# agimus-project/agimus_controller

Hardware: AMD Instinct MI355X
Metric: MPC steps/sec (horizon=100, Panda 7-DoF) (higher is better)
Workload: dtype f64; 1 GPU; Panda 7-DoF sine_wave_configuration_space, ocp_goal_reaching.yaml costs, horizon=100, dt=0.01, batch=1024 independent MPC instances per GPU (seed 1234+b), closed loop on own prediction; horizon=100, batch_per_gpu=1024, global_batch=1024, max_iter=10

## Files before the change

### agimus_controller_amd/csrc/agimus_hip.hip

```cpp

#include <hip/hip_runtime.h>

#include <algorithm>
#include <chrono>
#include <climits>
#include <cmath>
#include <cstddef>
#include <cstdio>
#include <cstdlib>
#include <cstring>
#include <string>
#include <vector>

#include "agx_kernels.hpp"

extern "C" int agx_cost_pairs_launch(int dest, void *stream, long long nodes, const DevModel *m, const DevOcp *o, const DevCostWide *w,
                                     const double *dts, const double *xs, const RefView *rv, double *out, double *auxs, const DevState *st,
                                     int phase, int sel, int which, const void *obs);
extern "C" int agx_cost_pairs_fill_launch(void *stream, const DevCostWide *w, const double *gw_item, double *traj, long long units, int stride);
extern "C" int agx_cost_pairs_fill_ring_launch(void *stream, const DevCostWide *w, const double *gw_item, double *traj, int B, int m_new, int end,
                                               int cap, int mirror, int stride);
extern "C" int agx_diag_iter_log_launch(void *stream, const DevState *st, int B, int it, int phase, agx_iter_record *rec, int *n, int capacity);
extern "C" int agx_diag_item_costs_launch(void *stream, int nv, int chain, const DevModel *m, const DevRows *rows2, int B, int T, const double *xs,
                                          const double *us, const RefView *rv, int R, double *cost, double *Lx, double *Lu, const void *obs);
// ... 359 lines not shown
      HIPCHK(hipGetLastError());
      return 0;
    }
    if constexpr (NV <= 7) {
      if (pair && o->riccati_mx && !forward)
        hipLaunchKernelGGL((agx::k_riccati_mx_pair_sweeps<NV>), dim3(16 * ((o->B + 7) / 8)), dim3(64), 0, o->stream, o->d_ocp, o->d_dt, o->d_qt,
                           o->d_aux, o->d_Kws, o->d_kws, o->d_dx, o->d_w, o->d_Kout, o->d_state, iter);
      else if (pair && o->riccati_mx)
        hipLaunchKernelGGL((agx::k_riccati_mx_pair<NV>), dim3(16 * ((o->B + 7) / 8)), dim3(64), 0, o->stream, o->d_ocp, o->d_dt, o->d_qt, o->d_aux,
                           o->d_Kws, o->d_kws, o->d_dx, o->d_w, o->d_Kout, o->d_state, iter);
      else if (pair)
        hipLaunchKernelGGL((agx::k_riccati_pair<NV>), dim3(2 * o->B), dim3(64), 0, o->stream, o->d_ocp, o->d_dt, o->d_qt, o->d_aux,
                           o->d_Kws, o->d_kws, o->d_dx, o->d_w, o->d_du, o->d_Kout, o->d_state, iter);
      else if (o->riccati_mx)
        hipLaunchKernelGGL((agx::k_riccati_mx<NV, false>), dim3(o->B), dim3(64), 0, o->stream, o->d_ocp, o->d_dt, qt, o->d_aux,
                           o->d_Kws, o->d_kws, o->d_dx, o->d_w, o->d_Kout, o->d_state, forward, 0);
      else
        hipLaunchKernelGGL((agx::k_riccati<NV, false>), dim3(o->B), dim3(64), 0, o->stream, o->d_ocp, o->d_dt, qt, o->d_aux,
                           o->d_Kws, o->d_kws, o->d_dx, o->d_w, o->d_du, o->d_Kout, o->d_state, forward, 0);
    } else {
      (void)pair; (void)iter;
      launch_riccati_blk<NV>(o, qt, forward, 0);
    }
    HIPCHK(hipGetLastError());
    return 0;
  });
}

agx::HostWords host_words(agx_ocp *o, bool line_search_counters, unsigned long long seq) {
  agx::HostWords hw{nullptr, nullptr, nullptr, nullptr, nullptr, nullptr, 0};
  if (!o->poll || !o->fold_publish || seq == 0) return hw;
  hw.done = o->h_ndone_dev + 0;
  if (line_search_counters) { hw.handed = o->h_ndone_dev + 6; hw.stale = o->h_ndone_dev + 7; }
  hw.carry = o->h_ndone_dev + 8;
  hw.packed = o->h_ndone_dev + 9;
  hw.seq = o->h_ndone_dev + 1;
  hw.stamp = seq;
  return hw;
}

double *first_block(const agx_ocp *o) {
  return (o->first_in_solve && o->poll && o->first_stride == o->nu + o->nu * o->nx + o->nx + 8) ? o->d_first : nullptr;
}

int launch_step(agx_ocp *o, int iter, int max_iter, int mode, bool with_node_kkt = true, bool with_step = true, unsigned long long seq = 0,
                bool pack = false) {
  if (o->T + 1 > 512) return fail("step kernel supports horizons up to 511 nodes");
  return dispatch(o->nv, o->chain, [&](auto NVc, auto CHc) -> int {
    constexpr int NV = decltype(NVc)::value;
    constexpr bool CH = decltype(CHc)::value;
    (void)CH;
    const long long nodes = (long long)o->B * (o->T + 1);
    double *xs_t = o->d_xs + (size_t)o->B * (o->T + 1) * o->nx, *us_t = o->d_us + (size_t)o->B * o->T * o->nu;
    if (with_node_kkt) {
      if constexpr (NV <= 7) {
        if (o->general)
          hipLaunchKernelGGL((agx::k_node_kkt_gen<NV>), dim3((int)((nodes + 63) / 64)), dim3(64), 0, o->stream, o->d_ocp, o->d_qt, o->d_aux,
                             o->d_auxg, o->d_dx, o->d_w, o->d_du, o->d_nodestat, o->d_state);
        else if (o->node_kkt_wide)
          hipLaunchKernelGGL((agx::k_node_kkt_ahead<NV>), dim3((int)((nodes + 7) / 8)), dim3(64), 0, o->stream, o->d_ocp, o->d_qt, o->d_aux,
                             o->d_dx, o->d_w, o->d_du, o->d_nodestat, o->d_state);
        else
          hipLaunchKernelGGL((agx::k_node_kkt<NV>), dim3((int)((nodes * 8 + 255) / 256)), dim3(256), 0, o->stream, o->d_ocp, o->d_qt, o->d_aux,
                             o->d_dx, o->d_w, o->d_du, o->d_nodestat, o->d_state);
      } else if (kGeneralRowsWg && o->general)
        HIPCHK((hipError_t)agx_general_kkt_launch((void *)o->stream, NV, nodes, o->d_ocp, o->d_qt, o->d_aux, o->d_auxg, o->d_dx, o->d_w, o->d_du,
                                                  o->d_nodestat, o->d_state));
      else
        hipLaunchKernelGGL((agx::k_node_kkt_big<NV>), dim3((int)((nodes + 1) / 2)), dim3(64), 0, o->stream, o->d_ocp, o->d_qt, o->d_aux,
                           o->d_dx, o->d_w, o->d_du, o->d_nodestat, o->d_state);
    }
    if (with_step)
      hipLaunchKernelGGL((agx::k_sqp_head<NV>), dim3(o->B), dim3(128), 0, o->stream, o->d_ocp, o->d_xs, o->d_us, o->d_dx, o->d_du, xs_t, us_t,
                         o->d_nodestat, o->d_state, iter, max_iter, mode, o->d_ndone, host_words(o, false, seq), o->d_Kout,
                         pack ? first_block(o) : nullptr, o->first_stride);
    HIPCHK(hipGetLastError());
    return 0;
  });
}

bool step_tail_path(const agx_ocp *o) {
  return o->step_tail && o->nv <= 7 && !o->has_con && !o->general && o->riccati_mx && o->node_kkt_wide && o->mx2_S < 2;
}
int launch_step_tail(agx_ocp *o, int iter, int max_iter, unsigned long long seq, bool pack) {
  if (o->T + 1 > 512) return fail("step kernel supports horizons up to 511 nodes");
  return dispatch(o->nv, o->chain, [&](auto NVc, auto CHc) -> int {
    constexpr int NV = decltype(NVc)::value;
    (void)CHc;
    if constexpr (NV <= 7) {
      double *xs_t = o->d_xs + (size_t)o->B * (o->T + 1) * o->nx, *us_t = o->d_us + (size_t)o->B * o->T * o->nu;
      hipLaunchKernelGGL((agx::k_step_tail<NV>), dim3(o->B), dim3(agx::kTailThreads), 0, o->stream, o->d_ocp, o->d_dt, o->d_qt, o->d_aux,
                         o->d_Kws, o->d_kws, o->d_xs, o->d_us, o->d_dx, o->d_w, o->d_du, xs_t, us_t, o->d_nodestat, o->d_state, iter,
                         max_iter, o->d_ndone, host_words(o, false, seq), o->d_Kout, pack ? first_block(o) : nullptr, o->first_stride);
      HIPCHK(hipGetLastError());
      o->step_tail_launches += 1;
      return 0;
    } else {
      (void)iter; (void)max_iter; (void)seq; (void)pack;
      return fail("the step tail serves the 7-joint capacity");
    }
  });
}

int launch_gains(agx_ocp *o, int gmode = 0) {
  if (o->nv <= 7 && o->T + 1 > 512) return fail("the sweeps stage the step lengths of up to 511 nodes in LDS: horizon too long");
  if (o->nv > 7 && !o->d_qt2) HIPCHK(o->own.device(&o->d_qt2, (size_t)o->B * (o->T + 1) * o->qt_size));
  return dispatch(o->nv, o->chain, [&](auto NVc, auto CHc) -> int {
    constexpr int NV = decltype(NVc)::value;
    if constexpr (NV <= 7) {
      if (o->riccati_mx)
        hipLaunchKernelGGL((agx::k_riccati_mx<NV, true>), dim3(o->B), dim3(64), 0, o->stream, o->d_ocp, o->d_dt, o->d_qt, o->d_aux, o->d_Kws,
                           o->d_kws, o->d_dx, o->d_w, o->d_Kout, o->d_state, 0, gmode);
      else
      hipLaunchKernelGGL((agx::k_riccati<NV, true>), dim3(o->B), dim3(64), 0, o->stream, o->d_ocp, o->d_dt, o->d_qt, o->d_aux, o->d_Kws,
                         o->d_kws, o->d_dx, o->d_w, o->d_du, o->d_Kout, o->d_state, 0, gmode);
    } else {
      const long long nodes = (long long)o->B * (o->T + 1);
      const int gsel = gmode == 0 ? 1 : gmode;
      hipLaunchKernelGGL((agx::k_sigma_tile_big<NV>), dim3((int)nodes), dim3(256), 0, o->stream, o->d_ocp, o->d_qt, o->d_qt2, o->d_aux);
      launch_riccati_blk<NV>(o, o->d_qt2, 0, gsel);
      if constexpr (NV > 16) {
        if (o->gains_mfma) {
          hipLaunchKernelGGL((agx::k_gains_to_u_mfma<NV>), dim3(o->B * o->T), dim3(64), 0, o->stream, o->d_ocp, o->d_aux, o->d_Kws, o->d_Kout,
                             o->d_state);
          HIPCHK(hipGetLastError());
          return 0;
        }
      }
      const long long units = (long long)o->B * o->T * 64;
      hipLaunchKernelGGL((agx::k_gains_to_u_big<NV>), dim3((int)((units + 255) / 256)), dim3(256), 0, o->stream, o->d_ocp, o->d_aux,
                         o->d_Kws, o->d_Kout, o->d_state);
    }
    HIPCHK(hipGetLastError());
    return 0;
  });
}

int reset_state(agx_ocp *o) {
  hipLaunchKernelGGL(agx::k_reset_state, dim3((o->B + 255) / 256), dim3(256), 0, o->stream, o->d_state, o->B, o->d_ndone);
  HIPCHK(hipGetLastError());
  return 0;
}

int launch_rollout(agx_ocp *o, int n_substeps, double dt_sub, const double *d_dist) {
  return dispatch(o->nv, o->chain, [&](auto NVc, auto CHc) -> int {
    constexpr int NV = decltype(NVc)::value;
    constexpr bool CH = decltype(CHc)::value;
    if (o->plant_set || o->minert_set)
      hipLaunchKernelGGL((agx::k_plant_rollout<NV, CH>), dim3((o->B + 63) / 64), dim3(64), 0, o->stream, o->d_model,
                         (const agx::PlantInertials<NV> *)(o->plant_set ? o->d_plant : o->d_minert), o->d_us, o->d_Kout, o->d_x0, d_dist, o->B, o->T,
                         n_substeps, dt_sub);
    else
      hipLaunchKernelGGL((agx::k_feedback_rollout<NV, CH>), dim3((o->B + 63) / 64), dim3(64), 0, o->stream, o->d_model, o->d_us, o->d_Kout, o->d_x0,
                         d_dist, o->B, o->T, n_substeps, dt_sub);
    HIPCHK(hipGetLastError());
    return 0;
  });
}

int prof_mark(agx_ocp *o, int kind, bool start) {
  if (!o->prof) return 0;
  if (o->prof_used == o->prof_ev.size()) {
    o->prof_ev.push_back(nullptr);
    HIPCHK(o->own.event(&o->prof_ev.back()));
  }
  HIPCHK(hipEventRecord(o->prof_ev[o->prof_used++], o->stream));
  if (start) o->prof_kind.push_back(kind);
  return 0;
}
int prof_collect(agx_ocp *o) {
  if (!o->prof || o->prof_used == 0) return 0;
  HIPCHK(hipStreamSynchronize(o->stream));
  for (size_t k = 0; k < o->prof_kind.size(); ++k) {
    float ms = 0.f;
    HIPCHK(hipEventElapsedTime(&ms, o->prof_ev[2 * k], o->prof_ev[2 * k + 1]));
    o->prof_ms[o->prof_kind[k]] += ms;
// ... 1895 lines not shown
```

### agimus_controller_amd/csrc/agx_host_handle.hpp

```cpp
#pragma once

#include <deque>

namespace {

thread_local std::string g_err;
int fail(const std::string &msg) {
  g_err = msg;
  return -1;
}
#define HIPCHK(expr)                                                                                      \
  do {                                                                                                    \
    hipError_t e_ = (expr);                                                                               \
    if (e_ != hipSuccess) return fail(std::string(#expr) + ": " + hipGetErrorString(e_));                \
  } while (0)

class DeviceOwner {
 public:
  DeviceOwner() = default;
  DeviceOwner(const DeviceOwner &) = delete;
  ~DeviceOwner() { for (const Held &h : held_) free_value(*h.field, h.kind); }
  template <class T> hipError_t device(T **field, size_t count, bool zero = false) { return device_bytes((void **)field, sizeof(T) * count, zero); }
  hipError_t device_bytes(void **field, size_t bytes, bool zero = false) {
    void *p = nullptr;
// ... 11 lines not shown
    const hipError_t e = hipEventCreateWithFlags(&ev, flags);
    return adopt((void **)field, (void *)ev, kEvent, e);
  }
  template <class T> void release(T *field) {
    for (Held &h : held_)
      if (h.field == (void **)field) {
        free_value(*h.field, h.kind);
        *h.field = nullptr;
        h = held_.back();
        held_.pop_back();
        return;
      }
  }

 private:
  enum Kind { kDevice, kPinned, kEvent };
  struct Held { void **field; Kind kind; };
  static void free_value(void *p, Kind kind) {
    if (p) (void)(kind == kDevice ? hipFree(p) : (kind == kPinned ? hipHostFree(p) : hipEventDestroy((hipEvent_t)p)));
  }
  hipError_t adopt(void **field, void *p, Kind kind, hipError_t e) {
    if (e != hipSuccess) return e;
    release(field);
    *field = p;
    held_.push_back({field, kind});
    return hipSuccess;
  }
  std::vector<Held> held_;
};

}

struct agx_model {
  DevModel h;
  int nvu = 0;
};

struct agx_ocp {
  DevModel hm;
  DevOcp ho;
  int nv = 0, nx = 0, nu = 0, T = 0, B = 0, tile = 0, stride = 0, device = 0;
  int nvu = 0, stride_u = 0;
  bool padded = false;
  std::vector<int> refmap[2];
  std::vector<double> reffill[2];
  std::vector<double> stage;
  std::vector<double> h_first_u;
  bool chain = false;
  std::vector<double> dt;
  hipStream_t stream = nullptr;
  bool own_stream = false;
  DevModel *d_model = nullptr;
  DevOcp *d_ocp = nullptr;
  double *d_dt = nullptr, *d_xs = nullptr, *d_us = nullptr, *d_x0 = nullptr, *d_tiles = nullptr;
  double *d_Kws = nullptr, *d_kws = nullptr, *d_Kout = nullptr, *d_dx = nullptr, *d_du = nullptr;
  double *d_Kws_lqr = nullptr, *d_kws_lqr = nullptr;
  bool admm_prefactor = true;
  double *d_qt = nullptr, *d_aux = nullptr, *d_w = nullptr, *d_nodestat = nullptr;
  bool has_con = false;
  std::vector<int> shift_nodes;
  int *d_shift_nodes = nullptr;
  bool general = false;
  double *d_auxg = nullptr;
  double *d_qt2 = nullptr, *d_cg = nullptr, *d_cjac = nullptr, *d_y = nullptr, *d_z = nullptr, *d_cx = nullptr, *d_admmstat = nullptr,
         *d_fac = nullptr,
         *d_segP = nullptr;
  bool admm_segments = true;
  int qt_size = 0, aux_size = 0;
  bool k1_lanes = true;
  bool lanes_ok = true;
  bool lanes_coll = false;
  bool cost_wide = false;
  DevCostWide hw{};
  DevCostWide *d_cw = nullptr;
  DevOcp *d_ocp_k1 = nullptr;
  int n_rows_all[2] = {0, 0};
  bool speculate = true;
  bool gains_mfma = true;
  bool riccati_mx = true;
  int mx2_S = 0;
  double *d_mx2_elem = nullptr, *d_mx2_bnd = nullptr, *d_mx2_cl = nullptr;
  bool k1_fused = true;
  bool node_kkt_wide = true;
  long long step_tail_launches = 0;
  bool step_tail = true;
  bool tile_carry = true;
  bool carry_static = false;
  bool carry_armed = false;
  int carry_k0 = 0;
  int head = 0;
  int n_carriable = -1;
  bool frames_uniform = true;
  double quorum_sqp = 1.0, quorum_qp = 1.0;
  bool con_lanes = true;
  bool con_wide = false;
  int con_cs = AGX_MAX_NC;
  bool admm_loop_always = false;
  bool admm_loop = true;
  int n_unfinished = 1 << 30;
  bool fold_publish = false;
  int n_cu = 256;
  bool no_empty = false;
  double *d_ref = nullptr;
  double *d_ref_back = nullptr;
  int *d_frames_back = nullptr;
  bool refs_pending = false, refs_pending_frames = false;
  hipStream_t copy_stream = nullptr;
  hipEvent_t ev_refs = nullptr, ev_snap = nullptr, ev_dl = nullptr;
  double *d_snap = nullptr;
  bool dl_pending = false;
  int *d_frames = nullptr;
  bool frames_set = false;
  DevState *d_state = nullptr;
  int *d_ndone = nullptr;
  unsigned long long *h_ndone = nullptr;
  unsigned long long *h_ndone_dev = nullptr;
  unsigned long long seq = 0;
  unsigned ls_handed = 0, ls_stale = 0;
  bool poll = true;
  double *d_first = nullptr, *h_first = nullptr;
  int first_stride = 0;
  bool first_in_solve = true;
  bool first_fresh = false;
  int n_packed = 0;
  long long first_served[2] = {0, 0};
  long long steps_carried = 0, steps_full = 0;
  long long early_exits = 0;
  double *d_scratch = nullptr;
  size_t scratch_bytes = 0;
  double *d_plant = nullptr;
  bool plant_set = false;
  std::vector<double> plant_stage;
  double *d_minert = nullptr;
  bool minert_set = false;
  std::vector<double> minert_stage;
  void *d_obs = nullptr;
  size_t obs_bytes = 0;
  bool obs_set = false;
  std::vector<double> obs_stage;
  RefView rv{};
  double *d_traj = nullptr, *d_pts = nullptr;
  double *d_sine = nullptr;
  int n_points = 0;
  std::vector<int> hidx;
  int *d_hidx = nullptr;
  int win_logical = -1;
  int win_k0 = 0;
  bool streamed = false;
  int st_cap = 0, st_span = 0, st_first = 0, st_end = 0;
  int st_chunk = 0;
  double *st_host[2] = {nullptr, nullptr}, *d_st_stage[2] = {nullptr, nullptr};
  hipEvent_t ev_st[2] = {nullptr, nullptr}, ev_st_solver = nullptr;
  bool st_used[2] = {false, false}, st_pending[2] = {false, false};
  int st_lo[2] = {0, 0};
  int st_next = 0;
  bool st_timing = false;
  std::deque<hipEvent_t> st_tev[2];
  size_t st_tev_used[2] = {0, 0};
  double st_tms[2] = {0.0, 0.0};
  long long st_tn[2] = {0, 0};
  long long st_joins = 0;
  agx::SineParams st_sp{};
  struct { int buf = -1, m = 0, end = 0; size_t used = 0; agx::SineParams sp{}; } st_last;
  hipEvent_t ev0 = nullptr, ev1 = nullptr, ev_done = nullptr;
  int last_max_iter = 0;
  int log_cap = 0;
// ... 111 lines not shown
```

### agimus_controller_amd/csrc/agx_kernels.hpp

```cpp
#pragma once

#include <type_traits>

#include "agx_device.hpp"

#include "agx_tiles.hpp"

namespace agx {

constexpr double kSigma = 1e-6;
constexpr double kRegMin = 1e-9;
constexpr double kRegMax = 1e9;

__device__ __forceinline__ void count_carriable(DevState &S, int *n_done) {
  const int c = (S.tiles_ok && S.preg == kRegMin) ? 1 : 0;
  if (c != S.carry_counted) { atomicAdd(n_done + 6, c - S.carry_counted); S.carry_counted = c; }
}

template <int NV, bool CHAIN, bool GEN = false, class... INST>
__global__ void __launch_bounds__(64) k_calc_diff(const DevModel *__restrict__ mp, const DevOcp *__restrict__ op,
                                                  const double *__restrict__ dts, const double *__restrict__ xs,
                                                  const double *__restrict__ us, RefView rv,
                                                  double *__restrict__ tiles, const DevState *__restrict__ st,
                                                  const INST *__restrict__... inst) {
// ... 296 lines not shown
  CostGen<NV> g;
  if constexpr (GEN) node_costs_general<NV, CHAIN, true, true>(m, o.rows[1], k, x, nullptr, ref_at(rv, b, T, T), frames_at(rv, b, T, T), c, g);
  qt[Q::cost] = c.cost;
AGX_UNROLL_NV
  for (int i = 0; i < NV; ++i) {
    qt[Q::gx + i] = c.Lq[i];
    qt[Q::gx + NV + i] = c.Lv[i];
    qt[Q::gw + i] = 0.0;
    qt[Q::f + i] = 0.0;
    qt[Q::f + NV + i] = 0.0;
    ax[A::Lvv + i] = c.Lvv[i];
    ax[A::Luu + i] = 0.0;
    ax[A::Lu + i] = 0.0;
AGX_UNROLL_NV
    for (int j = 0; j < NV; ++j) {
      qt[Q::Hqq + i * Q::LD + j] = c.Lqq[i][j];
      qt[Q::Hqv + i * Q::LD + j] = GEN ? g.Lqv[i][j] : 0.0;
      qt[Q::Hvv + i * Q::LD + j] = ((i == j) ? c.Lvv[i] : 0.0) + (GEN ? g.Lvvd[i][j] : 0.0);
      if constexpr (GEN) {
        double *ag = auxg + ((long long)b * (T + 1) + T) * (3 * A::B2);
        ag[i * A::LD + j] = g.Lqv[i][j];
        ag[A::B2 + i * A::LD + j] = g.Lvvd[i][j];
        ag[2 * A::B2 + i * A::LD + j] = 0.0;
      }
      qt[Q::Hqw + i * Q::LD + j] = 0.0;
      qt[Q::Hvw + i * Q::LD + j] = 0.0;
      qt[Q::Hww + i * Q::LD + j] = 0.0;
      ax[A::M + i * A::LD + j] = 0.0;
      ax[A::tq + i * A::LD + j] = 0.0;
      ax[A::tv + i * A::LD + j] = 0.0;
      ax[A::Lqq + i * A::LD + j] = c.Lqq[i][j];
    }
  }
}

template <int NV, bool CHAIN, bool GEN = false, class... OBS>
__global__ void __launch_bounds__(64) k_calc_qp_term(const DevModel *__restrict__ mp, const DevOcp *__restrict__ op,
                                                     const double *__restrict__ xs, RefView rv, double *__restrict__ qts,
                                                     double *__restrict__ auxs, const DevState *__restrict__ st,
                                                     double *__restrict__ auxg = nullptr, int phase = 0, const OBS *__restrict__... obs) {
  calc_qp_term_body<NV, CHAIN, GEN>(blockIdx.x * blockDim.x + threadIdx.x, mp, op, xs, rv, qts, auxs, st, auxg, phase, obs...);
}

__device__ __forceinline__ double wave_max(double v) {
#pragma unroll
  for (int off = 32; off > 0; off >>= 1) v = fmax(v, __shfl_xor(v, off, 64));
  return v;
}
__device__ __forceinline__ double wave_sum(double v) {
#pragma unroll
  for (int off = 32; off > 0; off >>= 1) v += __shfl_xor(v, off, 64);
  return v;
}

template <int K>
__device__ __forceinline__ double grid_col(double x) {
  double d = __builtin_amdgcn_mov_dpp(x, 0x150 + K, 0xf, 0xf, false);
  return __builtin_amdgcn_update_dpp(d, x, 0x150 + 8 + K, 0xf, 0xc, false);
}
template <class SET, int N>
__device__ __forceinline__ void prefetch_queue_settle(SET (&sets)[N]) {
  static_assert(sizeof(SET) % sizeof(double) == 0, "register sets of doubles");
#pragma unroll
  for (int i = 0; i < N; ++i) {
    double *p = reinterpret_cast<double *>(&sets[i]);
#pragma unroll
    for (int e = 0; e < (int)(sizeof(SET) / sizeof(double)); ++e) asm volatile("" : "+v"(p[e]));
  }
}
__device__ __forceinline__ void prefetch_group_begin() { __builtin_amdgcn_sched_barrier(0); }
__device__ __forceinline__ void prefetch_group_end() { __builtin_amdgcn_sched_barrier(0); }
constexpr int kMaxHorizon = 512;
__device__ __forceinline__ void stage_dts(double *__restrict__ s_dt, const double *__restrict__ dts, int T) {
  for (int i = threadIdx.x & 63; i < T; i += 64) s_dt[i] = dts[i];
  wave_lds_sync();
}
__device__ __forceinline__ double fast_rcp(double x) {
  double y = __builtin_amdgcn_rcp(x);
  y = y * (2.0 - x * y);
  y = y * (2.0 - x * y);
  return y;
}

struct FwdNoTap {
  __device__ __forceinline__ void start(int) const {}
  __device__ __forceinline__ void node(int, int, double, double, double) const {}
  __device__ __forceinline__ void done_to(int) const {}
};
template <int NV, class TAP = FwdNoTap>
__device__ __forceinline__ void riccati_forward(const DevOcp &o, const int b, const int T, const double *__restrict__ dts, const double *__restrict__ qb,
                                                const double *__restrict__ Kw, const double *__restrict__ kw,
                                                double *__restrict__ dxs, double *__restrict__ wss, const double *s_dt, const TAP tap = TAP()) {
  constexpr int NX = 2 * NV, TS = QT<NV>::SIZE;
  typedef QT<NV> Q;
  const int lane = threadIdx.x;
  const int r = lane >> 3, c = lane & 7;
  const bool in = (r < NV) && (c < NV);
  const int rr = r < NV ? r : 0, cc = c < NV ? c : 0;
  const double inm = in ? 1.0 : 0.0;
  double *dx = dxs + (long long)b * (T + 1) * NX, *ws = wss + (long long)b * T * NV;
  if (lane < NV) { dx[lane] = 0.0; dx[NV + lane] = 0.0; }
  tap.start(lane);
  __threadfence_block();
  double dq_r = 0.0, dv_r = 0.0, dq_c = 0.0, dv_c = 0.0;
  struct Gain { double kq, kv, kw, fq, fv; };
#ifndef AGX_FWD_DEPTH
#define AGX_FWD_DEPTH 8
#endif
  constexpr int FWD_DEPTH = AGX_FWD_DEPTH;
  auto load_gain = [&](Gain &g, int t) {
    const double *kr = Kw + ((long long)t * NV + rr) * NX;
    g.kq = kr[cc];
    g.kv = kr[NV + cc];
    g.kw = kw[(long long)t * NV + rr];
    const double *tl = qb + (long long)tile_slot(o, t) * TS;
    g.fq = tl[Q::f + rr];
    g.fv = tl[Q::f + NV + rr];
  };
  auto row_sum = [](double p) { p += dpp_xor1(p); p += dpp_xor2(p); p += dpp_xor4(p); return p; };
  auto fstep = [&](Gain &g, int t) {
    const double h = s_dt[t], h2 = h * h;
    double p = (g.kq * inm) * dq_c + (g.kv * inm) * dv_c;
    const double kwv = g.kw, fqc = g.fq, fvc = g.fv;
    p = row_sum(p);
    const double wv = -(kwv + p);
    const double nq = dq_r + h * dv_r + h2 * wv + fqc;
    const double nv2 = dv_r + h * wv + fvc;
    dq_r = nq; dv_r = nv2;
    dq_c = __shfl(nq, 8 * cc, 64);
    dv_c = __shfl(nv2, 8 * cc, 64);
    if (c == 0 && r < NV) {
      ws[(long long)t * NV + r] = wv;
      dx[(long long)(t + 1) * NX + r] = nq;
      dx[(long long)(t + 1) * NX + NV + r] = nv2;
      tap.node(t, r, wv, nq, nv2);
    }
    prefetch_group_begin();
    load_gain(g, t + FWD_DEPTH < T ? t + FWD_DEPTH : T - 1);
    prefetch_group_end();
  };
  int t = 0;
  for (int rem = T % FWD_DEPTH; rem > 0; --rem, ++t) {
    Gain g1;
    load_gain(g1, t);
    fstep(g1, t);
    tap.done_to(t + 1);
  }
  if (t < T) {
    Gain g[FWD_DEPTH];
#pragma unroll
    for (int i = 0; i < FWD_DEPTH; ++i) load_gain(g[i], t + i);
    prefetch_queue_settle(g);
    for (; t < T; t += FWD_DEPTH) {
#pragma unroll
      for (int i = 0; i < FWD_DEPTH; ++i) fstep(g[i], t + i);
      tap.done_to(t + FWD_DEPTH);
    }
  }
}

template <int NV>
struct FT {
  static constexpr int FW = 0, FQ = 56, FV = 112, RP = 168, PQ = 176, PV = 184, SIZE = 192;
};

template <int NV, bool GAINS, bool STORE = false>
__device__ __forceinline__ void riccati_body(const int b, const DevOcp *__restrict__ op, const double *__restrict__ dts,
                                             const double *__restrict__ qts, const double *__restrict__ auxs,
                                             double *__restrict__ Kws, double *__restrict__ kws,
                                             double *__restrict__ dxs, double *__restrict__ wss,
                                             double *__restrict__ dus, double *__restrict__ Kout,
                                             DevState *__restrict__ st, int forward, int gmode, int iter,
                                             double *__restrict__ facs = nullptr) {
  (void)dus;
  constexpr int gains_pass = GAINS ? 1 : 0;
  typedef AUX<NV> A;
  static_assert(NV <= 7, "the register-resident Riccati kernel maps an NV x NV block plus a gradient column onto an 8 x 8 lane grid");
  constexpr int NX = 2 * NV, TS = QT<NV>::SIZE;
  typedef QT<NV> Q;
  const DevOcp &o = *op;
  const int T = o.T, lane = threadIdx.x;
  DevState &S = st[b];
  bool bad_pivot = false;
  if (!gains_pass && (S.done || S.admm_conv)) return;
  if (gains_pass && (gmode == 1 || gmode == 4) && S.done) return;
  if (gains_pass && gmode == 2 && S.gains_iter == S.dir_iter) return;
  const double dreg = (gains_pass && gmode != 1 && gmode != 4) ? (S.solved ? S.dreg : S.gains_dreg) : S.dreg;
  if (gains_pass && gmode != 0 && lane == 0) S.gains_iter = (gmode == 1) ? iter : S.dir_iter;
  const double *qb = qts + (long long)b * (T + 1) * TS;
  const double *ab = auxs + (long long)b * (T + 1) * A::SIZE;
  double *Kw = Kws + (long long)b * T * NV * NX, *kw = kws + (long long)b * T * NV;
  double *Ko = GAINS ? Kout + (long long)b * T * NV * NX : nullptr;
  const double sig = GAINS ? kSigma : 0.0;
  const int r = lane >> 3, c = lane & 7;
  const bool in = (r < NV) && (c < NV);
  const int rc = in ? r * Q::LD + c : 0, cr = in ? c * Q::LD + r : 0;
  const int rr = r < NV ? r : 0, cc = c < NV ? c : 0;
  const double diag = (r == c) ? 1.0 : 0.0;
  const int col_lane = c;
  double Vqq, Vqv, Vvq, Vvv, vxq, vxv;
  {
    const double *tt = qb + (long long)T * TS;
    Vqq = in ? tt[Q::Hqq + rc] + (dreg + sig) * diag : 0.0;
    Vqv = in ? tt[Q::Hqv + rc] : 0.0;
    Vvq = in ? tt[Q::Hqv + cr] : 0.0;
    Vvv = in ? tt[Q::Hvv + rc] + (dreg + sig) * diag : 0.0;
    vxq = (r < NV) ? tt[Q::gx + rr] : 0.0;
    vxv = (r < NV) ? tt[Q::gx + NV + rr] : 0.0;
  }
  constexpr int kGridDepth = 4;
  struct Tile {
    double hqq, hqv, hvq, hvv, hqw, hvw, hwq, hwv, hww, gq, gv, gwr, fq, fv;
  };
  constexpr int AXN = 3 * A::B2;
  __shared__ double s_aux[GAINS ? 2 : 1][GAINS ? AXN : 1];
  double axr0 = 0.0, axr1 = 0.0, axr2 = 0.0;
  auto aux_fetch = [&](int t) {
    const double *al = ab + (long long)tile_slot(o, t) * A::SIZE + A::M;
    axr0 = (lane < AXN) ? al[lane] : 0.0;
    axr1 = (64 + lane < AXN) ? al[64 + lane] : 0.0;
    axr2 = (128 + lane < AXN) ? al[128 + lane] : 0.0;
  };
  auto aux_put = [&](int t) {
    double *sa = s_aux[GAINS ? (t & 1) : 0];
    if (lane < AXN) sa[lane] = axr0;
    if (64 + lane < AXN) sa[64 + lane] = axr1;
    if (128 + lane < AXN) sa[128 + lane] = axr2;
  };
  auto load_tile = [&](Tile &z, int t) {
    const double *tl = qb + (long long)tile_slot(o, t) * TS;
    z.hqq = tl[Q::Hqq + rc]; z.hqv = tl[Q::Hqv + rc]; z.hvq = tl[Q::Hqv + cr]; z.hvv = tl[Q::Hvv + rc];
    z.hqw = tl[Q::Hqw + rc]; z.hvw = tl[Q::Hvw + rc]; z.hwq = tl[Q::Hqw + cr]; z.hwv = tl[Q::Hvw + cr];
    z.hww = tl[Q::Hww + rc];
    if (!GAINS) {
      z.gq = tl[Q::gx + rr]; z.gv = tl[Q::gx + NV + rr]; z.gwr = tl[Q::gw + rr];
      z.fq = tl[Q::f + cc]; z.fv = tl[Q::f + NV + cc];
    }
  };
// ... 1410 lines not shown
```

### agimus_controller_amd/csrc/agx_step_tail.hpp

```cpp
#pragma once

namespace agx {

constexpr int kTailCap = 128;
constexpr int kTailThreads = 256;
constexpr int kHeadThreads = 128;

template <int NV>
struct FwdTailTap {
  double *s_dx, *s_w;
  int *s_prog;
  __device__ __forceinline__ void start(int lane) const {
    if (lane < NV) { s_dx[lane] = 0.0; s_dx[NV + lane] = 0.0; }
  }
  __device__ __forceinline__ void node(int t, int r, double wv, double nq, double nv2) const {
    if (t < kTailCap) {
      s_w[t * NV + r] = wv;
      s_dx[(t + 1) * 2 * NV + r] = nq;
      s_dx[(t + 1) * 2 * NV + NV + r] = nv2;
    }
  }
  __device__ __forceinline__ void done_to(int n) const {
    __builtin_amdgcn_fence(__ATOMIC_RELEASE, "workgroup");
    if (threadIdx.x == 0) __hip_atomic_store(s_prog, n, __ATOMIC_RELAXED, __HIP_MEMORY_SCOPE_WORKGROUP);
  }
};

template <int NV>
__global__ void __launch_bounds__(kTailThreads, 4) k_step_tail(const DevOcp *__restrict__ op, const double *__restrict__ dts,
                                                               const double *__restrict__ qts, const double *__restrict__ auxs,
                                                               const double *__restrict__ Kws, const double *__restrict__ kws,
                                                               const double *__restrict__ xs, const double *__restrict__ us,
                                                               double *dxs, double *wss, double *dus,
                                                               double *__restrict__ xs_t, double *__restrict__ us_t,
                                                               double *nodestat, DevState *__restrict__ st, int iter, int max_iter,
                                                               int *__restrict__ n_done, HostWords hw, const double *__restrict__ Kout,
                                                               double *__restrict__ first, int first_stride) {
  static_assert(NV <= 7, "one 8 x 8 lane grid per instance, eight lanes per node");
  constexpr int NX = 2 * NV, NU = NV;
  typedef QT<NV> Q;
  typedef AUX<NV> A;
  __shared__ double s_dt[kMaxHorizon];
  __shared__ double s_dx[(kTailCap + 1) * NX];
  __shared__ double s_w[kTailCap * NV];
  __shared__ double s_du[kTailCap * NV];
  __shared__ double s_ns[(kTailCap + 1) * 3];
  __shared__ int s_prog;
  __shared__ double red[8];
  __shared__ double s_words[8];
  __shared__ int flag;
  const DevOcp &o = *op;
  const int T = o.T, b = blockIdx.x, tid = threadIdx.x;
  DevState &S = st[b];
  if (S.done) {
    if (tid == 0) arrive_and_publish(n_done, hw);
    return;
  }
  if (tid == 0) s_prog = 0;
  __syncthreads();
  const int nxs = (T + 1) * NX, nus = T * NU;
  const long long ox = (long long)b * nxs, ou = (long long)b * nus;
  double *dxb = dxs + ox, *wb = wss + ou, *dub = dus + ou, *nsb = nodestat + (long long)b * (T + 1) * 4;
  if (tid < 64) {
    stage_dts(s_dt, dts, T);
    const double *qb = qts + (long long)b * (T + 1) * Q::SIZE;
    riccati_forward<NV>(o, b, T, dts, qb, Kws + (long long)b * T * NV * NX, kws + (long long)b * T * NV, dxs, wss, s_dt,
                        FwdTailTap<NV>{s_dx, s_w, &s_prog});
  } else {
    const int l8 = tid & 7, wave = tid >> 6;
    const double preg = S.preg, dreg = S.dreg;
    const bool jl = l8 < NV;
    const int jj = jl ? l8 : 0;
    const int n_groups = (T + 8) >> 3;
    for (int g = wave - 1; g < n_groups; g += 3) {
      const int t_lane = 8 * g + ((tid & 63) >> 3);
      const bool act = t_lane <= T;
      const int t = act ? t_lane : 0;
      const long long sid = (long long)b * (T + 1) + tile_slot(o, t);
      const double *qt = qts + sid * Q::SIZE;
      const double *ax = auxs + sid * A::SIZE;
      const double fq_l = qt[Q::f + jj], fv_l = qt[Q::f + NV + jj];
      const double cost = qt[Q::cost];
      double rM[8] = {}, rtq[8] = {}, rtv[8] = {}, rLqq[8] = {}, rLuu = 0.0, rLvv = 0.0;
      if (t < T) {
#pragma unroll
        for (int i = 0; i < NV; ++i) {
          rM[i] = ax[A::M + i * A::LD + l8]; rtq[i] = ax[A::tq + i * A::LD + l8]; rtv[i] = ax[A::tv + i * A::LD + l8];
        }
        rLuu = ax[A::Luu + l8];
      }
      if (t > 0) {
#pragma unroll
        for (int i = 0; i < NV; ++i) rLqq[i] = ax[A::Lqq + i * A::LD + l8];
        rLvv = ax[A::Lvv + l8];
      }
      const int need = 8 * g + 8 < T ? 8 * g + 8 : T;
      while (__hip_atomic_load(&s_prog, __ATOMIC_RELAXED, __HIP_MEMORY_SCOPE_WORKGROUP) < need) __builtin_amdgcn_s_sleep(2);
      __builtin_amdgcn_fence(__ATOMIC_ACQUIRE, "workgroup");
      double dq_l, dv_l, wj_l = 0.0;
      if (t <= kTailCap) { dq_l = s_dx[t * NX + jj]; dv_l = s_dx[t * NX + NV + jj]; }
      else { dq_l = dxb[t * NX + jj]; dv_l = dxb[t * NX + NV + jj]; }
      if (t < T) wj_l = t < kTailCap ? s_w[t * NV + jj] : wb[t * NV + jj];
      const double dq = jl ? dq_l : 0.0, dv = jl ? dv_l : 0.0;
      double kkt = 0.0, gap = 0.0;
      if (t < T) {
        const double wj = jl ? wj_l : 0.0;
        const double fq = jl ? fq_l : 0.0, fv = jl ? fv_l : 0.0;
        kkt = fmax(fabs(fq), fabs(fv));
        gap = fabs(fq) + fabs(fv);
        double pr[8];
#pragma unroll
        for (int i = 0; i < 8; ++i) pr[i] = (i < NV) ? rM[i] * wj + rtq[i] * dq + rtv[i] * dv : 0.0;
        const double du = transpose_reduce8(pr, l8);
        if (jl) {
          if (act) {
            dub[t * NV + l8] = du;
            if (t < kTailCap) s_du[t * NV + l8] = du;
          }
          kkt = fmax(kkt, fabs((rLuu + preg) * du));
        }
      }
      if (t > 0) {
        double pr[8];
AGX_UNROLL_NV
        for (int i = 0; i < 8; ++i) pr[i] = (i < NV) ? rLqq[i] * dq : 0.0;
        const double hq = transpose_reduce8(pr, l8);
        if (jl) kkt = fmax(kkt, fmax(fabs(hq + dreg * dq), fabs((rLvv + dreg) * dv)));
      }
      kkt = fmax(kkt, dpp_xor4(kkt)); kkt = fmax(kkt, dpp_xor2(kkt)); kkt = fmax(kkt, dpp_xor1(kkt));
      gap += dpp_xor4(gap); gap += dpp_xor2(gap); gap += dpp_xor1(gap);
      if (act && l8 == 0) {
        double *ns = nsb + t * 4;
        ns[0] = kkt; ns[1] = cost; ns[2] = gap; ns[3] = 0.0;
        if (t <= kTailCap) { s_ns[t * 3 + 0] = kkt; s_ns[t * 3 + 1] = cost; s_ns[t * 3 + 2] = gap; }
      }
    }
  }
  __syncthreads();

  const bool hd = tid < kHeadThreads;
  double px[kPrefX], pu[kPrefU];
#pragma unroll
  for (int k = 0; k < kPrefX; ++k) {
    const int e = tid + k * kHeadThreads;
    px[k] = (hd && e < nxs) ? xs[ox + e] : 0.0;
  }
#pragma unroll
  for (int k = 0; k < kPrefU; ++k) {
    const int e = tid + k * kHeadThreads;
    pu[k] = (hd && e < nus) ? us[ou + e] : 0.0;
  }
  auto dx_at = [&](int e) -> double { return e < (kTailCap + 1) * NX ? s_dx[e] : dxb[e]; };
  auto du_at = [&](int e) -> double { return e < kTailCap * NV ? s_du[e] : dub[e]; };
  constexpr int NK = NU * NX, FS = NU + NK + NX + 8;
  static_assert(FS <= kHeadThreads, "the record of the 7-joint capacity fits one stride of the head");
  const bool may_pack = first != nullptr && S.gains_iter == iter;
  auto record_element = [&](int e) -> double {
    if (e < NU) return us[ou + e];
    if (e < NU + NK) return Kout[(long long)b * T * NK + (e - NU)];
    return xs[ox + NX + (e - NU - NK)];
  };
  double prec = 0.0;
  if (may_pack && tid < FS - 8) prec = record_element(tid);
  if (hd) {
    double kkt = 0.0, csum = 0.0, gsum = 0.0, vsum = 0.0;
    for (int t = tid; t <= T; t += kHeadThreads) {
      if (t <= kTailCap) {
        kkt = fmax(kkt, s_ns[t * 3 + 0]);
        csum += s_ns[t * 3 + 1];
        gsum += s_ns[t * 3 + 2];
      } else {
        const double *ns = nsb + t * 4;
        kkt = fmax(kkt, ns[0]);
        csum += ns[1];
        gsum += ns[2];
      }
    }
    kkt = wave_max(kkt);
    csum = wave_sum(csum);
    gsum = wave_sum(gsum);
    vsum = wave_sum(vsum);
    if ((tid & 63) == 0) { red[tid >> 6] = kkt; red[2 + (tid >> 6)] = csum; red[4 + (tid >> 6)] = gsum; red[6 + (tid >> 6)] = vsum; }
  }
  __syncthreads();
  if (tid == 0) {
    double kk = fmax(red[0], red[1]);
    const double cc = red[2] + red[3], gg = red[4] + red[5], vv = red[6] + red[7];
    kk = fmax(kk, vv);
    const int dir_fail = S.dir_fail;
    S.carry = 0;
    if (dir_fail) kk = __builtin_nan("");
    S.kkt = kk; S.cost = cc; S.gap = gg; S.con = vv; S.merit = cc + o.mu_dyn * gg + o.mu_con * vv;
    S.qp_iters = 1;
    S.admm_conv = 0;
    S.dir_iter = iter;
    if (!(kk == kk)) S.flags |= 1;
    const bool conv = kk <= o.tol;
    int what = 0;
    if (conv) {
      S.solved = 1; S.done = 1; S.iter = iter; S.tiles_ok = 1; atomicAdd(n_done, 1);
      if (may_pack) {
        what = 2;
        s_words[0] = kk; s_words[1] = cc; s_words[2] = S.merit; s_words[3] = gg;
        s_words[4] = iter; s_words[5] = S.qp_iters; s_words[6] = 1; s_words[7] = S.flags;
      }
    } else {
      S.tiles_ok = 0;
      if (dir_fail) { S.flags |= 4; sqp_iteration_end(S, false, 1.0 / 512.0, iter, max_iter, n_done); }
      else {
        what = 1;
        S.searching = 1;
        S.ls_n = 0;
        double pr = S.preg, dr = S.dreg;
        bool stop;
        reg_schedule(1.0, pr, dr, stop);
        S.preg_trial = pr;
      }
    }
    flag = what;
    count_carriable(S, n_done);
    if (what != 2) arrive_and_publish(n_done, hw);
  }
  __syncthreads();
  if (flag == 2) {
    double *rec = first + (long long)b * first_stride;
    if (tid < FS) rec[tid] = tid < FS - 8 ? prec : s_words[tid - (FS - 8)];
    __syncthreads();
    if (tid == 0) {
      if (hw.seq) __threadfence_system();
      atomicAdd(n_done + 7, 1);
      arrive_and_publish(n_done, hw);
    }
    return;
  }
  if (!flag || !hd) return;
#pragma unroll
  for (int k = 0; k < kPrefX; ++k) {
    const int e = tid + k * kHeadThreads;
    if (e < nxs) xs_t[ox + e] = px[k] + 1.0 * dx_at(e);
  }
  for (int e = tid + kPrefX * kHeadThreads; e < nxs; e += kHeadThreads) xs_t[ox + e] = xs[ox + e] + 1.0 * dx_at(e);
#pragma unroll
  for (int k = 0; k < kPrefU; ++k) {
    const int e = tid + k * kHeadThreads;
    if (e < nus) us_t[ou + e] = pu[k] + 1.0 * du_at(e);
  }
  for (int e = tid + kPrefU * kHeadThreads; e < nus; e += kHeadThreads) us_t[ou + e] = us[ou + e] + 1.0 * du_at(e);
}

template <int NV>
__global__ void __launch_bounds__(64, 2) k_riccati_mx_pair_sweeps(const DevOcp *__restrict__ op, const double *__restrict__ dts,
                                                                  const double *__restrict__ qts, const double *__restrict__ auxs,
                                                                  double *__restrict__ Kws, double *__restrict__ kws,
                                                                  double *__restrict__ dxs, double *__restrict__ wss,
                                                                  double *__restrict__ Kout, DevState *__restrict__ st, int iter) {
  const int grp = blockIdx.x >> 4, w16 = blockIdx.x & 15;
  const int b = grp * 8 + (w16 & 7);
  if (b >= op->B) return;
  if (w16 >> 3)
    riccati_mx_body<NV, true>(b, op, dts, qts, auxs, Kws, kws, dxs, wss, Kout, st, 0, 1, iter);
  else
    riccati_mx_body<NV, false>(b, op, dts, qts, auxs, Kws, kws, dxs, wss, Kout, st, 0, 0, iter);
}

}
```

Measured before the change: 1.313 million MPC steps/s.

## Rework step-tail kernel: packed gain loads, SIMD-aware chain wave, deeper prefetch

The forward Riccati chain in the step-tail kernel now loads its per-node feedforward terms packed into one value per lane and spreads them with DPP moves. Its prefetch depth rises to 16. It picks which wave runs the serial chain from the hardware SIMD id and raises that wave's priority. Global stores of dx/w for the first nodes move off the critical chain into the node-consumer waves, and the final trajectory update now uses all 256 threads instead of 128. The aim is to shorten the serial forward recurrence latency, at the cost of more register pressure and added compile-time switches and trace instrumentation.

```diff
diff --git a/agimus_controller_amd/csrc/agimus_hip.hip b/agimus_controller_amd/csrc/agimus_hip.hip
--- a/agimus_controller_amd/csrc/agimus_hip.hip
+++ b/agimus_controller_amd/csrc/agimus_hip.hip
@@ -465,8 +465,36 @@
 bool step_tail_path(const agx_ocp *o) {
   return o->step_tail && o->nv <= 7 && !o->has_con && !o->general && o->riccati_mx && o->node_kkt_wide && o->mx2_S < 2;
 }
+#ifdef AGX_TAIL_TRACE
+static unsigned long long *g_tail_trace = nullptr;
+static long long g_tail_trace_words = 0;
+static int tail_trace_buffer(agx_ocp *o) {
+  const long long words = 2LL * o->B * agx::kTraceWords;
+  if (!o->d_tail_trace) {
+    HIPCHK(o->own.device(&o->d_tail_trace, (size_t)words));
+    HIPCHK(hipMemsetAsync(o->d_tail_trace, 0, words * sizeof(unsigned long long), o->stream));
+  }
+  g_tail_trace = o->d_tail_trace;
+  g_tail_trace_words = words;
+  return 0;
+}
+extern "C" long long agx_tail_trace_read(unsigned long long *dst, long long words) {
+  if (!g_tail_trace) return 0;
+  if (hipDeviceSynchronize() != hipSuccess) return -1;
+  const long long n = words < g_tail_trace_words ? words : g_tail_trace_words;
+  if (hipMemcpy(dst, g_tail_trace, n * sizeof(unsigned long long), hipMemcpyDeviceToHost) != hipSuccess) return -1;
+  if (hipMemset(g_tail_trace, 0, g_tail_trace_words * sizeof(unsigned long long)) != hipSuccess) return -1;
+  return n;
+}
+#define AGX_TAIL_TRACE_ARG , g_tail_trace
+#else
+#define AGX_TAIL_TRACE_ARG
+#endif
 int launch_step_tail(agx_ocp *o, int iter, int max_iter, unsigned long long seq, bool pack) {
   if (o->T + 1 > 512) return fail("step kernel supports horizons up to 511 nodes");
+#ifdef AGX_TAIL_TRACE
+  if (tail_trace_buffer(o)) return -1;
+#endif
   return dispatch(o->nv, o->chain, [&](auto NVc, auto CHc) -> int {
     constexpr int NV = decltype(NVc)::value;
     (void)CHc;
@@ -474,7 +502,7 @@
       double *xs_t = o->d_xs + (size_t)o->B * (o->T + 1) * o->nx, *us_t = o->d_us + (size_t)o->B * o->T * o->nu;
       hipLaunchKernelGGL((agx::k_step_tail<NV>), dim3(o->B), dim3(agx::kTailThreads), 0, o->stream, o->d_ocp, o->d_dt, o->d_qt, o->d_aux,
                          o->d_Kws, o->d_kws, o->d_xs, o->d_us, o->d_dx, o->d_w, o->d_du, xs_t, us_t, o->d_nodestat, o->d_state, iter,
-                         max_iter, o->d_ndone, host_words(o, false, seq), o->d_Kout, pack ? first_block(o) : nullptr, o->first_stride);
+                         max_iter, o->d_ndone, host_words(o, false, seq), o->d_Kout, pack ? first_block(o) : nullptr, o->first_stride AGX_TAIL_TRACE_ARG);
       HIPCHK(hipGetLastError());
       o->step_tail_launches += 1;
       return 0;
diff --git a/agimus_controller_amd/csrc/agx_host_handle.hpp b/agimus_controller_amd/csrc/agx_host_handle.hpp
--- a/agimus_controller_amd/csrc/agx_host_handle.hpp
+++ b/agimus_controller_amd/csrc/agx_host_handle.hpp
@@ -117,6 +117,9 @@
   double *d_mx2_elem = nullptr, *d_mx2_bnd = nullptr, *d_mx2_cl = nullptr;
   bool k1_fused = true;
   bool node_kkt_wide = true;
+#ifdef AGX_TAIL_TRACE
+  unsigned long long *d_tail_trace = nullptr;
+#endif
   long long step_tail_launches = 0;
   bool step_tail = true;
   bool tile_carry = true;
diff --git a/agimus_controller_amd/csrc/agx_kernels.hpp b/agimus_controller_amd/csrc/agx_kernels.hpp
--- a/agimus_controller_amd/csrc/agx_kernels.hpp
+++ b/agimus_controller_amd/csrc/agx_kernels.hpp
@@ -402,18 +402,28 @@
   return y;
 }
 
+#ifndef AGX_FWD_DEPTH
+#define AGX_FWD_DEPTH 8
+#endif
 struct FwdNoTap {
+  static constexpr int kDepth = AGX_FWD_DEPTH;
+  static constexpr bool kPacked = false;
+  __device__ __forceinline__ int lane() const { return threadIdx.x; }
   __device__ __forceinline__ void start(int) const {}
-  __device__ __forceinline__ void node(int, int, double, double, double) const {}
+  __device__ __forceinline__ bool node(int, int, double, double, double) const { return true; }
   __device__ __forceinline__ void done_to(int) const {}
 };
+template <bool PACKED>
+struct FwdGain { double kq, kv, kw, fq, fv; };
+template <>
+struct FwdGain<true> { double kq, kv, x; };
 template <int NV, class TAP = FwdNoTap>
 __device__ __forceinline__ void riccati_forward(const DevOcp &o, const int b, const int T, const double *__restrict__ dts, const double *__restrict__ qb,
                                                 const double *__restrict__ Kw, const double *__restrict__ kw,
                                                 double *__restrict__ dxs, double *__restrict__ wss, const double *s_dt, const TAP tap = TAP()) {
   constexpr int NX = 2 * NV, TS = QT<NV>::SIZE;
   typedef QT<NV> Q;
-  const int lane = threadIdx.x;
+  const int lane = tap.lane();
   const int r = lane >> 3, c = lane & 7;
   const bool in = (r < NV) && (c < NV);
   const int rr = r < NV ? r : 0, cc = c < NV ? c : 0;
@@ -423,25 +433,35 @@
   tap.start(lane);
   __threadfence_block();
   double dq_r = 0.0, dv_r = 0.0, dq_c = 0.0, dv_c = 0.0;
-  struct Gain { double kq, kv, kw, fq, fv; };
-#ifndef AGX_FWD_DEPTH
-#define AGX_FWD_DEPTH 8
-#endif
-  constexpr int FWD_DEPTH = AGX_FWD_DEPTH;
+  constexpr bool PACKED = TAP::kPacked;
+  typedef FwdGain<PACKED> Gain;
+  constexpr int FWD_DEPTH = TAP::kDepth;
+  double kw_n = 0.0, fq_n = 0.0, fv_n = 0.0;
   auto load_gain = [&](Gain &g, int t) {
     const double *kr = Kw + ((long long)t * NV + rr) * NX;
     g.kq = kr[cc];
     g.kv = kr[NV + cc];
-    g.kw = kw[(long long)t * NV + rr];
+    if constexpr (!PACKED) g.kw = kw[(long long)t * NV + rr];
     const double *tl = qb + (long long)tile_slot(o, t) * TS;
-    g.fq = tl[Q::f + rr];
-    g.fv = tl[Q::f + NV + rr];
+    if constexpr (PACKED) {
+      const int sel = c & 3;
+      const double *pk = kw + (long long)t * NV + rr, *pf = tl + Q::f + (sel == 2 ? NV : 0) + rr;
+      g.x = *((sel == 1 || sel == 2) ? pf : pk);
+    } else {
+      g.fq = tl[Q::f + rr];
+      g.fv = tl[Q::f + NV + rr];
+    }
+  };
+  auto unpack = [&](const Gain &g) {
+    if constexpr (PACKED) { kw_n = dpp_mov<0x00>(g.x); fq_n = dpp_mov<0x55>(g.x); fv_n = dpp_mov<0xAA>(g.x); }
   };
   auto row_sum = [](double p) { p += dpp_xor1(p); p += dpp_xor2(p); p += dpp_xor4(p); return p; };
-  auto fstep = [&](Gain &g, int t) {
+  auto fstep = [&](Gain &g, const Gain &g_next, int t) {
     const double h = s_dt[t], h2 = h * h;
     double p = (g.kq * inm) * dq_c + (g.kv * inm) * dv_c;
-    const double kwv = g.kw, fqc = g.fq, fvc = g.fv;
+    double kwv, fqc, fvc;
+    if constexpr (PACKED) { kwv = kw_n; fqc = fq_n; fvc = fv_n; }
+    else { kwv = g.kw; fqc = g.fq; fvc = g.fv; }
     p = row_sum(p);
     const double wv = -(kwv + p);
     const double nq = dq_r + h * dv_r + h2 * wv + fqc;
@@ -449,11 +469,13 @@
     dq_r = nq; dv_r = nv2;
     dq_c = __shfl(nq, 8 * cc, 64);
     dv_c = __shfl(nv2, 8 * cc, 64);
+    unpack(g_next);
     if (c == 0 && r < NV) {
-      ws[(long long)t * NV + r] = wv;
-      dx[(long long)(t + 1) * NX + r] = nq;
-      dx[(long long)(t + 1) * NX + NV + r] = nv2;
-      tap.node(t, r, wv, nq, nv2);
+      if (tap.node(t, r, wv, nq, nv2)) {
+        ws[(long long)t * NV + r] = wv;
+        dx[(long long)(t + 1) * NX + r] = nq;
+        dx[(long long)(t + 1) * NX + NV + r] = nv2;
+      }
     }
     prefetch_group_begin();
     load_gain(g, t + FWD_DEPTH < T ? t + FWD_DEPTH : T - 1);
@@ -463,7 +485,8 @@
   for (int rem = T % FWD_DEPTH; rem > 0; --rem, ++t) {
     Gain g1;
     load_gain(g1, t);
-    fstep(g1, t);
+    unpack(g1);
+    fstep(g1, g1, t);
     tap.done_to(t + 1);
   }
   if (t < T) {
@@ -471,9 +494,10 @@
 #pragma unroll
     for (int i = 0; i < FWD_DEPTH; ++i) load_gain(g[i], t + i);
     prefetch_queue_settle(g);
+    unpack(g[0]);
     for (; t < T; t += FWD_DEPTH) {
 #pragma unroll
-      for (int i = 0; i < FWD_DEPTH; ++i) fstep(g[i], t + i);
+      for (int i = 0; i < FWD_DEPTH; ++i) fstep(g[i], g[(i + 1) % FWD_DEPTH], t + i);
       tap.done_to(t + FWD_DEPTH);
     }
   }
diff --git a/agimus_controller_amd/csrc/agx_step_tail.hpp b/agimus_controller_amd/csrc/agx_step_tail.hpp
--- a/agimus_controller_amd/csrc/agx_step_tail.hpp
+++ b/agimus_controller_amd/csrc/agx_step_tail.hpp
@@ -1,28 +1,81 @@
 #pragma once
+
+#include "agx_tail_role.hpp"
+
+#ifndef AGX_TAIL_DEPTH
+#define AGX_TAIL_DEPTH 16
+#endif
+#ifndef AGX_TAIL_PACKED
+#define AGX_TAIL_PACKED 1
+#endif
+#ifndef AGX_TAIL_ROLE
+#define AGX_TAIL_ROLE 1
+#endif
+#ifndef AGX_TAIL_STORES
+#define AGX_TAIL_STORES 1
+#endif
+#ifndef AGX_TAIL_PRIO
+#define AGX_TAIL_PRIO 1
+#endif
 
 namespace agx {
 
 constexpr int kTailCap = 128;
 constexpr int kTailThreads = 256;
 constexpr int kHeadThreads = 128;
+constexpr int kTailPrefX = kPrefX / 2, kTailPrefU = kPrefU / 2;
+
+constexpr int kTraceWords = 256;
+#ifdef AGX_TAIL_TRACE
+struct TailTrace {
+  unsigned long long *rec;
+  __device__ __forceinline__ void put(int w, unsigned long long v) const {
+    if ((threadIdx.x & 63) == 0) rec[w] = v;
+  }
+  __device__ __forceinline__ void stamp(int w) const {
+    __builtin_amdgcn_sched_barrier(0);
+    put(w, wall_clock64());
+    __builtin_amdgcn_sched_barrier(0);
+  }
+  __device__ __forceinline__ void loads_arrived() const { asm volatile("s_waitcnt vmcnt(0)" ::: "memory"); }
+  __device__ __forceinline__ void hw_ids(int wave) const {
+    put(wave, (unsigned long long)__builtin_amdgcn_s_getreg((4 << 0) | (0 << 6) | (31 << 11)) |
+                  ((unsigned long long)__builtin_amdgcn_s_getreg((20 << 0) | (0 << 6) | (31 << 11)) << 32));
+  }
+};
+#else
+struct TailTrace {
+  __device__ __forceinline__ void put(int, unsigned long long) const {}
+  __device__ __forceinline__ void stamp(int) const {}
+  __device__ __forceinline__ void loads_arrived() const {}
+  __device__ __forceinline__ void hw_ids(int) const {}
+};
+#endif
 
 template <int NV>
 struct FwdTailTap {
+  static constexpr int kDepth = AGX_TAIL_DEPTH;
+  static constexpr bool kPacked = AGX_TAIL_PACKED != 0;
   double *s_dx, *s_w;
   int *s_prog;
+  TailTrace trace;
+  __device__ __forceinline__ int lane() const { return threadIdx.x & 63; }
   __device__ __forceinline__ void start(int lane) const {
     if (lane < NV) { s_dx[lane] = 0.0; s_dx[NV + lane] = 0.0; }
   }
-  __device__ __forceinline__ void node(int t, int r, double wv, double nq, double nv2) const {
+  __device__ __forceinline__ bool node(int t, int r, double wv, double nq, double nv2) const {
     if (t < kTailCap) {
       s_w[t * NV + r] = wv;
       s_dx[(t + 1) * 2 * NV + r] = nq;
       s_dx[(t + 1) * 2 * NV + NV + r] = nv2;
-    }
+      return AGX_TAIL_STORES == 0;
+    }
+    return true;
   }
   __device__ __forceinline__ void done_to(int n) const {
     __builtin_amdgcn_fence(__ATOMIC_RELEASE, "workgroup");
-    if (threadIdx.x == 0) __hip_atomic_store(s_prog, n, __ATOMIC_RELAXED, __HIP_MEMORY_SCOPE_WORKGROUP);
+    if ((threadIdx.x & 63) == 0) __hip_atomic_store(s_prog, n, __ATOMIC_RELAXED, __HIP_MEMORY_SCOPE_WORKGROUP);
+    if (n <= 111) trace.stamp(16 + n);
   }
 };
 
@@ -35,7 +88,11 @@
                                                                double *__restrict__ xs_t, double *__restrict__ us_t,
                                                                double *nodestat, DevState *__restrict__ st, int iter, int max_iter,
                                                                int *__restrict__ n_done, HostWords hw, const double *__restrict__ Kout,
-                                                               double *__restrict__ first, int first_stride) {
+                                                               double *__restrict__ first, int first_stride
+#ifdef AGX_TAIL_TRACE
+                                                               , unsigned long long *trace_buf
+#endif
+                                                               ) {
   static_assert(NV <= 7, "one 8 x 8 lane grid per instance, eight lanes per node");
   constexpr int NX = 2 * NV, NU = NV;
   typedef QT<NV> Q;
@@ -46,6 +103,7 @@
   __shared__ double s_du[kTailCap * NV];
   __shared__ double s_ns[(kTailCap + 1) * 3];
   __shared__ int s_prog;
+  __shared__ int s_simd[4];
   __shared__ double red[8];
   __shared__ double s_words[8];
   __shared__ int flag;
@@ -56,29 +114,53 @@
     if (tid == 0) arrive_and_publish(n_done, hw);
     return;
   }
-  if (tid == 0) s_prog = 0;
+#ifdef AGX_TAIL_TRACE
+  const TailTrace trace{trace_buf + ((long long)(iter & 1) * gridDim.x + b) * kTraceWords};
+#else
+  const TailTrace trace{};
+#endif
+  const int wave = __builtin_amdgcn_readfirstlane(tid >> 6);
+  if (tid == 0) { s_prog = 0; trace.stamp(8); }
+  if ((tid & 63) == 0) {
+    s_simd[wave] = (int)__builtin_amdgcn_s_getreg((4 << 0) | (4 << 6) | (1 << 11));
+    trace.hw_ids(wave);
+  }
   __syncthreads();
+#if AGX_TAIL_ROLE
+  const int chain_wave = __builtin_amdgcn_readfirstlane(tail_chain_wave(s_simd[0], s_simd[1], s_simd[2], s_simd[3], (b >> 8) & 3));
+#else
+  const int chain_wave = 0;
+#endif
+  const int rank = tail_node_rank(wave, chain_wave);
+  if (tid == 0) trace.put(9, (unsigned long long)chain_wave);
   const int nxs = (T + 1) * NX, nus = T * NU;
   const long long ox = (long long)b * nxs, ou = (long long)b * nus;
   double *dxb = dxs + ox, *wb = wss + ou, *dub = dus + ou, *nsb = nodestat + (long long)b * (T + 1) * 4;
-  if (tid < 64) {
+  if (rank < 0) {
+#if AGX_TAIL_PRIO
+    __builtin_amdgcn_s_setprio(3);
+#endif
     stage_dts(s_dt, dts, T);
     const double *qb = qts + (long long)b * (T + 1) * Q::SIZE;
     riccati_forward<NV>(o, b, T, dts, qb, Kws + (long long)b * T * NV * NX, kws + (long long)b * T * NV, dxs, wss, s_dt,
-                        FwdTailTap<NV>{s_dx, s_w, &s_prog});
+                        FwdTailTap<NV>{s_dx, s_w, &s_prog, trace});
+#if AGX_TAIL_PRIO
+    __builtin_amdgcn_s_setprio(0);
+#endif
   } else {
-    const int l8 = tid & 7, wave = tid >> 6;
+    const int l8 = tid & 7;
     const double preg = S.preg, dreg = S.dreg;
     const bool jl = l8 < NV;
     const int jj = jl ? l8 : 0;
     const int n_groups = (T + 8) >> 3;
-    for (int g = wave - 1; g < n_groups; g += 3) {
+    for (int g = rank; g < n_groups; g += 3) {
       const int t_lane = 8 * g + ((tid & 63) >> 3);
       const bool act = t_lane <= T;
       const int t = act ? t_lane : 0;
       const long long sid = (long long)b * (T + 1) + tile_slot(o, t);
       const double *qt = qts + sid * Q::SIZE;
       const double *ax = auxs + sid * A::SIZE;
+      if (g < 32) trace.stamp(128 + 4 * g);
       const double fq_l = qt[Q::f + jj], fv_l = qt[Q::f + NV + jj];
       const double cost = qt[Q::cost];
       double rM[8] = {}, rtq[8] = {}, rtv[8] = {}, rLqq[8] = {}, rLuu = 0.0, rLvv = 0.0;
@@ -95,12 +177,22 @@
         rLvv = ax[A::Lvv + l8];
       }
       const int need = 8 * g + 8 < T ? 8 * g + 8 : T;
+      if (g < 32) trace.stamp(128 + 4 * g + 1);
       while (__hip_atomic_load(&s_prog, __ATOMIC_RELAXED, __HIP_MEMORY_SCOPE_WORKGROUP) < need) __builtin_amdgcn_s_sleep(2);
       __builtin_amdgcn_fence(__ATOMIC_ACQUIRE, "workgroup");
+      if (g < 32) trace.stamp(128 + 4 * g + 2);
+      trace.loads_arrived();
+      if (g < 32) trace.stamp(128 + 4 * g + 3);
       double dq_l, dv_l, wj_l = 0.0;
       if (t <= kTailCap) { dq_l = s_dx[t * NX + jj]; dv_l = s_dx[t * NX + NV + jj]; }
       else { dq_l = dxb[t * NX + jj]; dv_l = dxb[t * NX + NV + jj]; }
       if (t < T) wj_l = t < kTailCap ? s_w[t * NV + jj] : wb[t * NV + jj];
+#if AGX_TAIL_STORES
+      if (act && jl) {
+        if (t > 0 && t <= kTailCap) { dxb[t * NX + l8] = dq_l; dxb[t * NX + NV + l8] = dv_l; }
+        if (t < T && t < kTailCap) wb[t * NV + l8] = wj_l;
+      }
+#endif
       const double dq = jl ? dq_l : 0.0, dv = jl ? dv_l : 0.0;
       double kkt = 0.0, gap = 0.0;
       if (t < T) {
@@ -136,19 +228,20 @@
       }
     }
   }
+  trace.stamp(4 + wave);
   __syncthreads();
 
   const bool hd = tid < kHeadThreads;
-  double px[kPrefX], pu[kPrefU];
-#pragma unroll
-  for (int k = 0; k < kPrefX; ++k) {
-    const int e = tid + k * kHeadThreads;
-    px[k] = (hd && e < nxs) ? xs[ox + e] : 0.0;
-  }
-#pragma unroll
-  for (int k = 0; k < kPrefU; ++k) {
-    const int e = tid + k * kHeadThreads;
-    pu[k] = (hd && e < nus) ? us[ou + e] : 0.0;
+  double px[kTailPrefX], pu[kTailPrefU];
+#pragma unroll
+  for (int k = 0; k < kTailPrefX; ++k) {
+    const int e = tid + k * kTailThreads;
+    px[k] = e < nxs ? xs[ox + e] : 0.0;
+  }
+#pragma unroll
+  for (int k = 0; k < kTailPrefU; ++k) {
+    const int e = tid + k * kTailThreads;
+    pu[k] = e < nus ? us[ou + e] : 0.0;
   }
   auto dx_at = [&](int e) -> double { return e < (kTailCap + 1) * NX ? s_dx[e] : dxb[e]; };
   auto du_at = [&](int e) -> double { return e < kTailCap * NV ? s_du[e] : dub[e]; };
@@ -230,22 +323,24 @@
       if (hw.seq) __threadfence_system();
       atomicAdd(n_done + 7, 1);
       arrive_and_publish(n_done, hw);
+      trace.stamp(10);
     }
     return;
   }
-  if (!flag || !hd) return;
-#pragma unroll
-  for (int k = 0; k < kPrefX; ++k) {
-    const int e = tid + k * kHeadThreads;
+  if (!flag) return;
+#pragma unroll
+  for (int k = 0; k < kTailPrefX; ++k) {
+    const int e = tid + k * kTailThreads;
     if (e < nxs) xs_t[ox + e] = px[k] + 1.0 * dx_at(e);
   }
-  for (int e = tid + kPrefX * kHeadThreads; e < nxs; e += kHeadThreads) xs_t[ox + e] = xs[ox + e] + 1.0 * dx_at(e);
-#pragma unroll
-  for (int k = 0; k < kPrefU; ++k) {
-    const int e = tid + k * kHeadThreads;
+  for (int e = tid + kTailPrefX * kTailThreads; e < nxs; e += kTailThreads) xs_t[ox + e] = xs[ox + e] + 1.0 * dx_at(e);
+#pragma unroll
+  for (int k = 0; k < kTailPrefU; ++k) {
+    const int e = tid + k * kTailThreads;
     if (e < nus) us_t[ou + e] = pu[k] + 1.0 * du_at(e);
   }
-  for (int e = tid + kPrefU * kHeadThreads; e < nus; e += kHeadThreads) us_t[ou + e] = us[ou + e] + 1.0 * du_at(e);
+  for (int e = tid + kTailPrefU * kTailThreads; e < nus; e += kTailThreads) us_t[ou + e] = us[ou + e] + 1.0 * du_at(e);
+  if (tid == 0) trace.stamp(10);
 }
 
 template <int NV>
diff --git a/agimus_controller_amd/csrc/agx_tail_role.hpp b/agimus_controller_amd/csrc/agx_tail_role.hpp
--- /dev/null
+++ b/agimus_controller_amd/csrc/agx_tail_role.hpp
@@ -0,0 +1,19 @@
+#pragma once
+
+#if defined(__HIPCC__) || defined(__CUDACC__)
+#define AGX_ROLE_HD __host__ __device__
+#else
+#define AGX_ROLE_HD
+#endif
+
+namespace agx {
+
+AGX_ROLE_HD constexpr int tail_chain_wave(int s0, int s1, int s2, int s3, int want) {
+  return ((s0 & 3) == (want & 3)) ? 0 : ((s1 & 3) == (want & 3)) ? 1 : ((s2 & 3) == (want & 3)) ? 2 : ((s3 & 3) == (want & 3)) ? 3 : 0;
+}
+
+AGX_ROLE_HD constexpr int tail_node_rank(int wave, int chain_wave) {
+  return wave == chain_wave ? -1 : wave - (wave > chain_wave ? 1 : 0);
+}
+
+}
```

New measurement: 1.324 million MPC steps/s (median of 6 runs). About the same (+0.9%).
